# shahruk10/kaldi-tflite

Hardware: AMD Instinct MI355X
Metric: x-vectors/sec (10 s @16 kHz) (higher is better)
Workload: dtype f16mx

## Files before the change

kaldi-tflite_amd/csrc/tdnn_mx.hip:

```cpp
#include "tdnn_mx_common.h"

#define MXP_ROWS 256
__global__ __launch_bounds__(MXP_ROWS) void mx_planes_kernel(const float* __restrict__ src, int64_t T, int64_t ld, int D,
                                                             const int32_t* __restrict__ lens, char* __restrict__ xh,
                                                             char* __restrict__ xl4, char* __restrict__ x4, char* __restrict__ xs) {
    __shared__ float tile[MXP_ROWS * 33];
    const int b = blockIdx.z, c = blockIdx.y, nch = gridDim.y;
    const int64_t t0 = (int64_t)blockIdx.x * MXP_ROWS;
    const int64_t len = lens ? (int64_t)lens[b] : T;
    if (t0 >= len) return;
    const int rows = (int)(len - t0 < MXP_ROWS ? len - t0 : MXP_ROWS);
    const int tid = threadIdx.x;
    const float* base = src + ((int64_t)b * T + t0) * ld + c * 32;
    const bool vec = (ld & 3) == 0 && ((uintptr_t)src & 15) == 0 && c * 32 + 32 <= ld;
#pragma unroll
    for (int k = 0; k < 8; ++k) {
        const int q = k * MXP_ROWS + tid, r = q >> 3, e4 = (q & 7) * 4;
        if (r < rows) {
            float v[4];
            if (vec) {
                const f32x4 t = *reinterpret_cast<const f32x4*>(base + (int64_t)r * ld + e4);
                const int nd = D - (c * 32 + e4);
                v[0] = nd > 0 ? t.x : 0.0f; v[1] = nd > 1 ? t.y : 0.0f; v[2] = nd > 2 ? t.z : 0.0f; v[3] = nd > 3 ? t.w : 0.0f;
            } else {
#pragma unroll
                for (int e = 0; e < 4; ++e) v[e] = (c * 32 + e4 + e < D) ? base[(int64_t)r * ld + e4 + e] : 0.0f;
            }
#pragma unroll
            for (int e = 0; e < 4; ++e) tile[r * 33 + e4 + e] = __builtin_amdgcn_fmed3f(v[e], -65504.0f, 65504.0f);
        }
    }
    __syncthreads();
    const int64_t rec0 = ((int64_t)b * nch + c) * T + t0;
    u32x4 hp[4];
    if (tid < rows) {
        float v[32];
#pragma unroll
        for (int e = 0; e < 32; ++e) v[e] = tile[tid * 33 + e];
        u32x4 l4, h4;
        unsigned sw;
        mx_encode32(v, hp, l4, h4, sw);
        *reinterpret_cast<u32x4*>(xl4 + (rec0 + tid) * 16) = l4;
        *reinterpret_cast<u32x4*>(x4 + (rec0 + tid) * 16) = h4;
        *reinterpret_cast<unsigned*>(xs + (rec0 + tid) * 4) = sw;
    }
    __syncthreads();
    unsigned* himg = reinterpret_cast<unsigned*>(tile);
    if (tid < rows) {
#pragma unroll
        for (int k = 0; k < 4; ++k) *reinterpret_cast<u32x4*>(himg + tid * 20 + k * 4) = hp[k];
    }
    __syncthreads();
#pragma unroll
    for (int k = 0; k < 4; ++k) {
        const int q = k * MXP_ROWS + tid, r = q >> 2;
        if (r < rows)
            *reinterpret_cast<u32x4*>(xh + rec0 * 64 + (int64_t)q * 16) = *reinterpret_cast<const u32x4*>(himg + r * 20 + (q & 3) * 4);
    }
}

extern "C" int ktf_mx_planes(const float* src, int64_t B, int64_t T, int32_t D, int64_t ld_src, const int32_t* lens, void* xh,
                             void* xl4, void* x4, void* xs, void* stream) {
    KTF_REQUIRE(B >= 0 && T >= 0 && D > 0 && ld_src >= D, "ktf_mx_planes: bad size");
    if (B == 0 || T == 0) return KTF_OK;
    KTF_REQUIRE(src && xh && xl4 && x4 && xs, "ktf_mx_planes: null argument");
    const int nch = (D + 31) / 32;
    KTF_REQUIRE(B < 65536 && nch < 65536, "ktf_mx_planes: B and D / 32 must be below 65536");
    hipLaunchKernelGGL(mx_planes_kernel, dim3((unsigned)((T + MXP_ROWS - 1) / MXP_ROWS), (unsigned)nch, (unsigned)B), dim3(MXP_ROWS), 0,
                       (hipStream_t)stream, src, T, ld_src, (int)D, lens, (char*)xh, (char*)xl4, (char*)x4, (char*)xs);
    KTF_CHECK_LAUNCH("ktf_mx_planes");
    return KTF_OK;
}

template <int ACT, int OUT, bool PADK, bool FLAT = false>
__device__ __forceinline__ void mx_tile(const MxParams& p, const int id, int mtiles, int ntiles, int gtiles, double* __restrict__ stats,
                                        unsigned char* rsm) {
    static_assert(!FLAT || OUT != MX_OUT_F32, "flat row tiles: plane output or fused pooling");
#define MX_ARG_BATCH()                                                                                                                     \
    asm volatile("" ::"s"(p.xh), "s"(p.wh), "s"(p.T), "s"(p.nss), "s"(p.nk), "s"(p.nctx), "s"(p.nch_in), "s"(p.ctx_pk[0]), "s"(p.ctx_pk[1]), \
                 "s"(p.t_div_m), "s"(p.t_div_s), "s"(p.start), "s"(p.sub), "s"(p.cut))
    const int xcd = id & 7, slot = id >> 3;
    const int g = (slot / ntiles) * 8 + xcd;
    const int nt = slot - (slot / ntiles) * ntiles;
    if (g >= gtiles) return;
    const int b = FLAT ? 0 : g / mtiles, mt = FLAT ? g : g - b * mtiles;
    const int n0 = nt * 256, t0 = FLAT ? 0 : mt * 256;
    const int tid = threadIdx.x, lane = tid & 63;
    const int wave = __builtin_amdgcn_readfirstlane(tid >> 6);
    const int wm = wave >> 2, wn = wave & 3;
    const int R0 = mt * 256;
    int len, out_len;
    [[maybe_unused]] bool dense = false;
    if constexpr (FLAT) {
        const int total = p.row_starts[mtiles];
        MX_ARG_BATCH();
        if (R0 >= total) return;
        len = (int)p.T;
        out_len = total - R0 < 256 ? total - R0 : 256;
        dense = total == mtiles * len;
    } else {
        len = p.lens ? p.lens[b] : (int)p.T;
        MX_ARG_BATCH();
        out_len = len - p.cut - p.start <= 0 ? 0 : (len - p.cut - p.start + p.sub - 1) / p.sub;
        if (t0 >= out_len) return;
    }
    const int lenm1 = len - 1;
    const int64_t ub = FLAT ? 0 : (int64_t)b * p.nch_in * p.T;
    const int nkp = p.nss * 4;
    const __amdgpu_buffer_rsrc_t r_xh = mx_rsrc_pinned(p.xh + (ub - MX_KQ_BIAS) * 64);
    const __amdgpu_buffer_rsrc_t r_wh = mx_rsrc_pinned(p.wh + (int64_t)nt * nkp * MX_TILE);
    const __amdgpu_buffer_rsrc_t r_wq = mx_rsrc_pinned(p.wq + (int64_t)nt * p.nss * MX_WQ_BLOCK);

    unsigned a_cb[2];
    int a_row[2];
#pragma unroll
    for (int i = 0; i < 2; ++i) {
        const int q = i * 512 + tid;
        const int row = q >> 2;
        a_cb[i] = (unsigned)(((q & 3) ^ ((4 - ((row >> 2) & 3)) & 3)) * 16);
        a_row[i] = p.start + (t0 + row) * p.sub;
    }
    [[maybe_unused]] int a_lm1[2] = {lenm1, lenm1}, s_lm1 = lenm1;
    int s_row = p.start + (t0 + lane + 64 * (wave & 3)) * p.sub;
    [[maybe_unused]] unsigned a_ub[2] = {0u, 0u}, s_ub = 0u;
    [[maybe_unused]] auto flat_row = [&](int m) -> i32x4 {
        if (dense) {
            const int R = R0 + m;
            if (m >= out_len) return i32x4{-1, 0, 1, 0};
            const int bb = p.t_div_m ? (int)(__umulhi((unsigned)R, p.t_div_m) >> p.t_div_s) : R;
            return i32x4{R, R - bb * len, len, bb};
        }
        return reinterpret_cast<const i32x4*>(p.row_map)[R0 + m];
    };
    const unsigned long long cpk0 = p.ctx_pk[0], cpk1 = p.ctx_pk[1];
#define MX_CTX(ci_) ((int)(signed char)(((ci_) < 8 ? cpk0 : cpk1) >> (((ci_) & 7) * 8)))
    [[maybe_unused]] bool interior = false;
    if constexpr (FLAT) {
        i32x4 er[3];
        const int mr[3] = {tid >> 2, (512 + tid) >> 2, lane + 64 * (wave & 3)};
        if (dense) {
#pragma unroll
            for (int i = 0; i < 3; ++i) er[i] = flat_row(mr[i]);
        } else {
#pragma unroll
            for (int i = 0; i < 3; ++i) er[i] = reinterpret_cast<const i32x4*>(p.row_map)[R0 + mr[i]];
        }
#pragma unroll
        for (int i = 0; i < 2; ++i) {
            a_row[i] = er[i].y;
            a_lm1[i] = er[i].z - 1;
            a_ub[i] = er[i].x < 0 ? 0u : (unsigned)(er[i].x - er[i].y) * (unsigned)p.nch_in;
        }
        s_row = er[2].y;
        s_lm1 = er[2].z - 1;
        s_ub = er[2].x < 0 ? 0u : (unsigned)(er[2].x - er[2].y) * (unsigned)p.nch_in;
    }
    const unsigned vw = (unsigned)tid * 16u;
    const int wave_k0 = (int)(unsigned)(size_t)(lds_ptr_t*)(rsm + wave * 1024);
    [[maybe_unused]] const int wave_k = wave_k0;
#define MX_LDS_AT(off_, c_) ((lds_ptr_t*)(size_t)(unsigned)((off_) + (c_)))
    int kb[5], ko[5];
    kb[0] = MX_KQ_BIAS;
    ko[0] = MX_CTX(0);
#define MX_DMA_A_E(ks_, e_, n_)                                                                                        \
    {                                                                                                                  \
        int r_ = a_row[n_] + ko[e_];                                                                                   \
        const int hi_ = FLAT ? a_lm1[n_] : lenm1;                                                                      \
        r_ = r_ < 0 ? 0 : (r_ > hi_ ? hi_ : r_);                                                                       \
        const unsigned vo_ = ((FLAT ? a_ub[n_] : 0u) + (unsigned)r_) * 64u + a_cb[n_];                                 \
        __builtin_amdgcn_raw_ptr_buffer_load_lds(r_xh, MX_LDS_AT(wave_k, ((ks_) & 1) * MX_STAGE + (n_) * 8192), 16, vo_, kb[e_] << 6, 0, 0); \
    }
#define MX_DMA_A_I(ks_, e_, n_)                                                                                        \
    __builtin_amdgcn_raw_ptr_buffer_load_lds(r_xh, MX_LDS_AT(wave_k, ((ks_) & 1) * MX_STAGE + (n_) * 8192), 16, (n_) ? va1 : va0, \
                                             (kb[e_] + ko[e_]) << 6, 0, 0);
#define MX_DMA_A(ks_, e_, n_) { if constexpr (INTERIOR) MX_DMA_A_I(ks_, e_, n_) else MX_DMA_A_E(ks_, e_, n_) }
#define MX_DMA_W(ks_, n_)                                                                                              \
    __builtin_amdgcn_raw_ptr_buffer_load_lds(r_wh, MX_LDS_AT(wave_k, ((ks_) & 1) * MX_STAGE + MX_TILE + (n_) * 8192), 16, vw, \
                                             (ks_) * MX_TILE + (n_) * 8192, 0, 0);
    MX_DMA_W(0, 0) MX_DMA_W(0, 1) MX_DMA_A_E(0, 0, 0) MX_DMA_A_E(0, 0, 1)
    const __amdgpu_buffer_rsrc_t r_xl4 = mx_rsrc_pinned(p.xl4 + (ub - MX_KQ_BIAS) * 16);
    const __amdgpu_buffer_rsrc_t r_x4 = mx_rsrc_pinned(p.x4 + (ub - MX_KQ_BIAS) * 16);
    const __amdgpu_buffer_rsrc_t r_xs = mx_rsrc_pinned(p.xs + (ub - MX_KQ_BIAS) * 4);
    if constexpr (FLAT) {
        if (p.nctx == 1 && MX_CTX(0) == 0) {
            interior = true;
        } else if (out_len == 256) {
            const i32x4 e0 = flat_row(0), e1 = flat_row(255);
            interior = __builtin_amdgcn_readfirstlane(e0.w) == __builtin_amdgcn_readfirstlane(e1.w) &&
                       __builtin_amdgcn_readfirstlane(e0.y) + MX_CTX(0) >= 0 &&
                       __builtin_amdgcn_readfirstlane(e1.y) + MX_CTX(p.nctx - 1) <= __builtin_amdgcn_readfirstlane(e1.z) - 1;
        }
    }
    [[maybe_unused]] const unsigned va0 = (a_ub[0] + (unsigned)a_row[0]) * 64u + a_cb[0], va1 = (a_ub[1] + (unsigned)a_row[1]) * 64u + a_cb[1];
    [[maybe_unused]] const unsigned vs16 = (s_ub + (unsigned)s_row) * 16u, vs4 = (s_ub + (unsigned)s_row) * 4u;

    const int sa_k0 = (int)(unsigned)(size_t)(lds_ptr_t*)(rsm + (wave & 3) * 1024 + (wave >> 2) * 4096);
    const int sa_ks0 = (int)(unsigned)(size_t)(lds_ptr_t*)(rsm + (wave & 3) * 256 + (wave >> 2) * 1024);
    const bool wave_hi = wave >= 4;

    int* const tkb = reinterpret_cast<int*>(rsm + MX_KQ_OFF);
    int* const tko = tkb + (nkp + 4);

#define MX_DMA_SA(n_)                                                                                                  \
    {                                                                                                                  \
        constexpr int plane_ = ((n_) < 4 ? (n_) : 0) >> 1, h_ = (n_) < 4 ? ((n_) & 1) : (n_) - 4;                      \
        unsigned rec_ = 0u;                                                                                            \
        int so_;                                                                                                       \
        if constexpr (INTERIOR) {                                                                                      \
            so_ = sk_b[h_] + sk_o[h_];                                                                                 \
        } else {                                                                                                       \
            int r_ = s_row + sk_o[h_];                                                                                 \
            const int hi_ = FLAT ? s_lm1 : lenm1;                                                                      \
            r_ = r_ < 0 ? 0 : (r_ > hi_ ? hi_ : r_);                                                                   \
            rec_ = (FLAT ? s_ub : 0u) + (unsigned)r_;                                                                  \
            so_ = sk_b[h_];                                                                                            \
        }                                                                                                              \
        if ((n_) < 4) {                                                                                                \
            __builtin_amdgcn_raw_ptr_buffer_load_lds(plane_ ? r_x4 : r_xl4, MX_LDS_AT(sa_k, MX_SA_OFF + plane_ * 16384 + h_ * 8192), 16, \
                                                     INTERIOR ? vs16 : rec_ * 16u, so_ << 4, 0, 0);                    \
        } else {                                                                                                       \
            __builtin_amdgcn_raw_ptr_buffer_load_lds(r_xs, MX_LDS_AT(sa_ks, MX_SA_OFF + 32768 + h_ * 2048), 4, INTERIOR ? vs4 : rec_ * 4u, so_ << 2, 0, 0); \
        }                                                                                                              \
    }
#define MX_DMA_SW(ss_, n_)                                                                                             \
    __builtin_amdgcn_raw_ptr_buffer_load_lds(r_wq, MX_LDS_AT(wave_k, MX_SW_OFF + (n_) * 8192), 16, vw, (ss_) * MX_WQ_BLOCK + (n_) * 8192, 0, 0);

    f32x4 acc[8][4];
    const int r16 = lane & 15, q4 = lane >> 4;
    const int fr = (4 - ((r16 >> 2) & 3)) & 3;
    const int coff = ((q4 ^ fr) << 4);
    const int a_row_off = (wm * 128 + r16) * 64 + coff;
    const int b_row_off = (wn * 64 + r16) * 64 + coff;
    const int klim = PADK ? p.nk : nkp;

    auto kloop = [&](auto itag) {
        constexpr bool INTERIOR = decltype(itag)::value;
        {
            unsigned char* const prm_w = rsm + MX_PRM_OFF + (wave & 3) * 256;
            const unsigned vcol = (unsigned)(n0 + (wave & 3) * 64 + lane) * 4u;
            const float* const vec0 = wave_hi ? p.scale : p.bias;
            if (vec0) __builtin_amdgcn_raw_ptr_buffer_load_lds(mx_rsrc(vec0, p.units * 4), (lds_ptr_t*)(prm_w + (wave_hi ? 1024 : 0)), 4, vcol, 0, 0, 0);
            else reinterpret_cast<float*>(prm_w + (wave_hi ? 1024 : 0))[lane] = wave_hi ? 1.0f : 0.0f;
            if (!wave_hi) {
                if (p.shift) __builtin_amdgcn_raw_ptr_buffer_load_lds(mx_rsrc(p.shift, p.units * 4), (lds_ptr_t*)(prm_w + 2048), 4, vcol, 0, 0, 0);
                else reinterpret_cast<float*>(prm_w + 2048)[lane] = 0.0f;
            }
        }
        for (int k = tid; k < nkp + 4; k += 512) {
            const int kk = k + 1 < p.nk ? k + 1 : 0;
            const int ch = kk / p.nctx, ci = kk - ch * p.nctx;
            tkb[k] = ch * (int)p.T + MX_KQ_BIAS;
            tko[k] = MX_CTX(ci);
        }
        {
            int ch = 0, ci = 0;
#pragma unroll
            for (int e = 1; e <= 4; ++e) {
                if (++ci == p.nctx) { ci = 0; ++ch; }
                const bool real = e < p.nk;
                kb[e] = (real ? ch * (int)p.T : 0) + MX_KQ_BIAS;
                ko[e] = real ? MX_CTX(ci) : MX_CTX(0);
            }
        }
#pragma unroll
        for (int i = 0; i < 8; ++i)
#pragma unroll
            for (int j = 0; j < 4; ++j) acc[i][j] = f32x4{0.0f, 0.0f, 0.0f, 0.0f};
        for (int ss = 0; ss < p.nss; ++ss) {
            i32x4 tb_n, to_n;
            int sk_b[2], sk_o[2];
            int wave_k = wave_k0, sa_k = sa_k0, sa_ks = sa_ks0;
            asm volatile("" : "+s"(wave_k), "+s"(sa_k), "+s"(sa_ks));
#pragma unroll
            for (int j = 0; j < 4; ++j) {
                const int ks = 4 * ss + j;
                if (j == 1 || j == 2) asm volatile("s_waitcnt vmcnt(6)" ::: "memory");
                else if (j == 0) asm volatile("s_waitcnt vmcnt(0) lgkmcnt(0)" ::: "memory");
                else asm volatile("s_waitcnt vmcnt(0)" ::: "memory");
                __builtin_amdgcn_s_barrier();
                asm volatile("" ::: "memory");
                const bool live = PADK ? ks < p.nk : true;
#define MX_NEXT() ({ int k1_ = ks + 1; asm volatile("" : "+s"(k1_)); k1_ < klim; })
                const unsigned char* sa = rsm + (ks & 1) * MX_STAGE;
                const unsigned char* sw = sa + MX_TILE;
                hfrag8 bh[4];
                hfrag8 a_cur, a_nx1;
                if (live) {
#pragma unroll
                    for (int jj = 0; jj < 4; ++jj) bh[jj] = *reinterpret_cast<const hfrag8*>(sw + b_row_off + jj * 1024);
                    a_cur = *reinterpret_cast<const hfrag8*>(sa + a_row_off);
                    a_nx1 = *reinterpret_cast<const hfrag8*>(sa + a_row_off + 1024);
                }
                __builtin_amdgcn_sched_barrier(0);
                if (MX_NEXT()) { MX_DMA_A(ks + 1, j + 1, 0) MX_DMA_A(ks + 1, j + 1, 1) }
                __builtin_amdgcn_sched_barrier(0);
#pragma unroll
                for (int i = 0; i < 8; ++i) {
                    if (live) {
                        acc[i][0] = __builtin_amdgcn_mfma_f32_16x16x32_f16(a_cur, bh[0], acc[i][0], 0, 0, 0);
                        __builtin_amdgcn_sched_barrier(0);
                        hfrag8 a_nx2 = a_nx1;
                        if (i < 6) a_nx2 = *reinterpret_cast<const hfrag8*>(sa + a_row_off + (i + 2) * 1024);
#pragma unroll
                        for (int jj = 1; jj < 4; ++jj) acc[i][jj] = __builtin_amdgcn_mfma_f32_16x16x32_f16(a_cur, bh[jj], acc[i][jj], 0, 0, 0);
                        a_cur = a_nx1;
                        a_nx1 = a_nx2;
                    }
                    __builtin_amdgcn_sched_barrier(0);
                    if (i == 0) { if (MX_NEXT()) MX_DMA_W(ks + 1, 0) }
                    if (i == 1) { if (MX_NEXT()) MX_DMA_W(ks + 1, 1) }
                    if (j == 0) {
                        if (i == 1) {
                            sk_b[0] = wave_hi ? kb[1] : kb[0]; sk_o[0] = wave_hi ? ko[1] : ko[0];
                            sk_b[1] = wave_hi ? kb[3] : kb[2]; sk_o[1] = wave_hi ? ko[3] : ko[2];
                        }
                        if (i == 2) MX_DMA_SA(0)
                        if (i == 3) MX_DMA_SA(1)
                        if (i == 4) MX_DMA_SA(2)
                        if (i == 5) MX_DMA_SA(3)
                        if (i == 6) MX_DMA_SA(4)
                        if (i == 7) MX_DMA_SA(5)
                    }
                    if (j == 1) {
                        if (i == 2) MX_DMA_SW(ss, 0)
                        if (i == 3) MX_DMA_SW(ss, 1)
                        if (i == 4) MX_DMA_SW(ss, 2)
                        if (i == 5) MX_DMA_SW(ss, 3)
                        if (i == 6) MX_DMA_SW(ss, 4)
                        if (i == 7) MX_DMA_SW(ss, 5)
                    }
                    if (j == 2 && i == 3) {
                        tb_n = *reinterpret_cast<const i32x4*>(tkb + 4 * ss + 4);
                        to_n = *reinterpret_cast<const i32x4*>(tko + 4 * ss + 4);
                    }
                    __builtin_amdgcn_sched_barrier(0);
                }
#undef MX_NEXT
            }
            __builtin_amdgcn_sched_barrier(0);
            {
                int tl;
                asm volatile("v_mbcnt_lo_u32_b32 %0, -1, 0\n\tv_mbcnt_hi_u32_b32 %0, -1, %0" : "=v"(tl));
                const int sw_rec = ((tl & 63) >> 4) * 256 + wn * 64 + (tl & 15);
                const int sa_rec = ((tl & 63) >> 4) * 256 + wm * 128 + (tl & 15);
                unsigned o_a16 = MX_SA_OFF + sa_rec * 16, o_a4 = MX_SA_OFF + 32768 + sa_rec * 4;
                asm volatile("" : "+v"(o_a16), "+v"(o_a4));
                const unsigned char* const pa16 = rsm + o_a16;
                const unsigned char* const pa4 = rsm + o_a4;
                unsigned o_w16 = MX_SW_OFF + sw_rec * 16, o_w8 = MX_SW_OFF + 32768 + sw_rec * 8, o_w4 = MX_SW_OFF + 40960 + sw_rec * 4;
                asm volatile("" : "+v"(o_w16), "+v"(o_w8), "+v"(o_w4));
                const unsigned char* const pw16 = rsm + o_w16;
                const unsigned char* const pw8 = rsm + o_w8;
                const unsigned char* const pw4 = rsm + o_w4;
                u32x4 w4[4], wl6a[4];
                u32x2 wl6b[4];
                unsigned wsc[4];
#pragma unroll
                for (int jj = 0; jj < 4; ++jj) {
                    w4[jj] = *reinterpret_cast<const u32x4*>(pw16 + jj * 256);
                    wl6a[jj] = *reinterpret_cast<const u32x4*>(pw16 + 16384 + jj * 256);
                    wl6b[jj] = *reinterpret_cast<const u32x2*>(pw8 + jj * 128);
                    wsc[jj] = *reinterpret_cast<const unsigned*>(pw4 + jj * 64);
                }
                u32x4 l_n = *reinterpret_cast<const u32x4*>(pa16);
                u32x4 h_n = *reinterpret_cast<const u32x4*>(pa16 + 16384);
                unsigned s_n = *reinterpret_cast<const unsigned*>(pa4);
#pragma unroll
                for (int i = 0; i < 8; ++i) {
                    const u32x4 l = l_n, h = h_n;
                    const unsigned asc = s_n;
                    if (i < 7) {
                        l_n = *reinterpret_cast<const u32x4*>(pa16 + (i + 1) * 256);
                        h_n = *reinterpret_cast<const u32x4*>(pa16 + 16384 + (i + 1) * 256);
                        s_n = *reinterpret_cast<const unsigned*>(pa4 + (i + 1) * 64);
                    }
                    const i32x8 al = i32x8{(int)l.x, (int)l.y, (int)l.z, (int)l.w, 0, 0, 0, 0};
                    const i32x8 ah = i32x8{(int)h.x, (int)h.y, (int)h.z, (int)h.w, 0, 0, 0, 0};
#pragma unroll
                    for (int jj = 0; jj < 4; ++jj) {
                        const i32x8 bw = i32x8{(int)w4[jj].x, (int)w4[jj].y, (int)w4[jj].z, (int)w4[jj].w, 0, 0, 0, 0};
                        acc[i][jj] = __builtin_amdgcn_mfma_scale_f32_16x16x128_f8f6f4(al, bw, acc[i][jj], 4, 4, 0, asc, 0, wsc[jj]);
                    }
#pragma unroll
                    for (int jj = 0; jj < 4; ++jj) {
                        const i32x8 bw = i32x8{(int)wl6a[jj].x, (int)wl6a[jj].y, (int)wl6a[jj].z, (int)wl6a[jj].w, (int)wl6b[jj].x, (int)wl6b[jj].y, 0, 0};
                        acc[i][jj] = __builtin_amdgcn_mfma_scale_f32_16x16x128_f8f6f4(ah, bw, acc[i][jj], 4, 2, 1, asc, 1, wsc[jj]);
                    }
                    if (i == 3) {
                        kb[0] = kb[4];
                        ko[0] = ko[4];
#pragma unroll
                        for (int e = 0; e < 4; ++e) {
                            kb[e + 1] = __builtin_amdgcn_readfirstlane(tb_n[e]);
                            ko[e + 1] = __builtin_amdgcn_readfirstlane(to_n[e]);
                        }
                    }
                    __builtin_amdgcn_sched_barrier(0);
                }
            }
        }
    };
    if constexpr (FLAT) {
        if (interior) kloop(std::true_type{});
        else kloop(std::false_type{});
    } else {
        kloop(std::false_type{});
    }
#undef MX_DMA_A
#undef MX_DMA_A_E
#undef MX_DMA_A_I
#undef MX_DMA_W
#undef MX_DMA_SA
#undef MX_DMA_SW
#undef MX_ARG_BATCH
#undef MX_LDS_AT
#undef MX_CTX

#include "tdnn_mx_epilogue.inc"
}

template <int ACT, int OUT, bool PADK, bool FLAT = false>
__global__ __launch_bounds__(512) void tdnn_mx_kernel(MxParams p, int mtiles, int ntiles, int gtiles, double* __restrict__ stats) {
    extern __shared__ __attribute__((aligned(16))) unsigned char rsm[];
    mx_tile<ACT, OUT, PADK, FLAT>(p, blockIdx.x, mtiles, ntiles, gtiles, stats, rsm);
}

static int mx_launch(const void* xh, const void* xl4, const void* x4, const void* xs, int64_t B, int64_t T, const int32_t* lens,
                     const KtfTdnnDesc* d, const void* wh, const void* wq, const float* bias, const float* scale, const float* shift,
                     void* yh, void* yl4, void* y4, void* ys, float* yf, int64_t ldy, double* stats, void* stream, const char* who,
                     const int32_t* row_starts = nullptr, const int32_t* row_map = nullptr) {
    KTF_REQUIRE(d && wh && wq, "%s: null argument", who);
    KTF_REQUIRE(d->gemm == KTF_GEMM_F16MX, "%s: needs KTF_GEMM_F16MX", who);
    KTF_REQUIRE(B >= 0 && T >= 0 && B < 65536, "%s: bad size", who);
    KTF_REQUIRE(B == 0 || T == 0 || (xh && xl4 && x4 && xs), "%s: null argument", who);
    if (const int rc = tdnn_check_desc(d, scale, shift, who); rc != KTF_OK) return rc;
    KTF_REQUIRE(d->subsampling <= 64, "%s: subsampling %d outside [1,64]", who, d->subsampling);
    const bool plain = !d->valid && d->subsampling == 1;
    KTF_REQUIRE(plain || !stats, "%s: the fused pooling takes SAME padding without subsampling", who);
    KTF_REQUIRE(d->act == KTF_ACT_NONE || d->act == KTF_ACT_RELU, "%s: fuses ReLU or no activation", who);
    KTF_REQUIRE(T * (int64_t)d->din_pad * 2 < (1ll << 31) - (1ll << 20), "%s: T * din_pad too large", who);
    KTF_REQUIRE((((int64_t)d->din_pad / 32 * d->nctx + 3) / 4) * 4 <= MX_KQ_MAX_STEPS || (d->flags & KTF_TDNN_MX_LOADER), "%s: more than %d K-steps (din_pad / 32 * contexts)", who, MX_KQ_MAX_STEPS);
    if (B == 0 || T == 0 || ktf_tdnn_out_len(T, d) <= 0) return KTF_OK;
    const int outs = (yh ? 1 : 0) + (yf ? 1 : 0) + (stats ? 1 : 0);
    KTF_REQUIRE(outs == 1, "%s: exactly one of the plane / fp32 / pooled outputs", who);
    if (yh) KTF_REQUIRE(yl4 && y4 && ys, "%s: a plane output needs all four planes", who);
    if (yf) KTF_REQUIRE(ldy >= d->units, "%s: ldy < units", who);
    if (B == 0 || T == 0) return KTF_OK;
    MxParams p;
    memset(&p, 0, sizeof(p));
    p.xh = (const char*)xh; p.xl4 = (const char*)xl4; p.x4 = (const char*)x4; p.xs = (const char*)xs;
    p.lens = lens; p.wh = (const char*)wh; p.wq = (const char*)wq; p.bias = bias; p.scale = scale; p.shift = shift;
    p.yh = (char*)yh; p.yl4 = (char*)yl4; p.y4 = (char*)y4; p.ys = (char*)ys; p.yf = yf; p.ldy = ldy; p.T = T;
    p.units = d->units; p.nch_in = d->din_pad / 32; p.nctx = d->nctx; p.nk = p.nch_in * d->nctx; p.nss = (p.nk + 3) / 4;
    p.nch_out = (d->units + 31) / 32;
    p.sub = d->subsampling;
    p.start = (d->valid && d->ctx[0] < 0) ? -d->ctx[0] : 0;
    p.cut = (d->valid && d->ctx[d->nctx - 1] > 0) ? d->ctx[d->nctx - 1] : 0;
    p.Tout = ktf_tdnn_out_len(T, d);
    if (p.Tout <= 0) return KTF_OK;
    KTF_REQUIRE(plain || !(d->flags & KTF_TDNN_MX_LOADER), "%s: the loader-wave kernel takes SAME padding without subsampling", who);
    const bool loader = (d->flags & KTF_TDNN_MX_LOADER) != 0;
    const PoolSlots pool = (row_starts && !loader) ? pool_flat128() : pool_slots_mx(d->flags);
    p.stat_slots = (stats && (d->flags & KTF_TDNN_DET_STATS)) ? (int32_t)pool.slots(T) : 0;
    for (int i = 0; i < d->nctx; ++i) {
        KTF_REQUIRE(d->ctx[i] >= -128 && d->ctx[i] <= 127, "%s: context offsets outside [-128, 127]", who);
        p.ctx_pk[i >> 3] |= (unsigned long long)(unsigned char)(signed char)d->ctx[i] << ((i & 7) * 8);
    }
    hipStream_t st = (hipStream_t)stream;
    const int o = stats ? MX_OUT_STATS : (yf ? MX_OUT_F32 : MX_OUT_PLANES);
    if (loader) {
        const int rc = mxl_launch(p, B, d->act, o, stats, st);
        if (rc != KTF_OK) return rc;
        KTF_CHECK_LAUNCH(who);
        return KTF_OK;
    }
    if (row_starts) {
        KTF_REQUIRE(row_map && plain && o != MX_OUT_F32 && !loader, "%s: flat row tiles take the row table, SAME padding, no subsampling, a plane or pooled output", who);
        KTF_REQUIRE(B <= 4095 && B * T * (int64_t)p.nch_in * 64 < (1ll << 32) - (1ll << 20) && B * T < (1ll << 31) / (p.nch_out > 0 ? p.nch_out : 1),
                    "%s: flat row tiles need B <= 4095 and B * T * din_pad * 2 < 2^32", who);
        p.row_starts = row_starts; p.row_map = row_map;
        if (T > 1) {
            uint32_t l = 0;
            while ((1ull << l) < (uint64_t)T) ++l;
            p.t_div_m = (uint32_t)((1ull << (31 + l)) / (uint64_t)T + 1);
            p.t_div_s = l - 1;
        }
        const int ntiles = ktf_cdiv(d->units, 256);
        const int64_t ftiles = ktf_cdiv(B * T, 256);
        const int64_t fblocks = grouped_blocks(ftiles, ntiles);
        tdnn_pick<MX_OUT_STATS, MX_OUT_PLANES>(o, [&](auto O) {
            tdnn_pick<KTF_ACT_RELU, KTF_ACT_NONE>(d->act, [&](auto A) {
                tdnn_pick<true, false>((p.nk & 3) != 0, [&](auto PADK) {
                    tdnn_launch_kernel<tdnn_mx_kernel<A, O, PADK, true>>("tdnn_mx_kernel<flat>", dim3((unsigned)fblocks), dim3(512), MX_LDS_TOTAL(p.nss * 4),
                                                                         MX_LDS_TOTAL(MX_KQ_MAX_STEPS), st, p, (int)B, ntiles, (int)ftiles, stats);
                });
            });
        });
        KTF_CHECK_LAUNCH(who);
        return KTF_OK;
    }
    const int mtiles = ktf_cdiv(p.Tout, 256), ntiles = ktf_cdiv(d->units, 256);
    const int64_t gtiles = B * mtiles;
    const int64_t nblocks = grouped_blocks(gtiles, ntiles);
    tdnn_pick<KTF_ACT_RELU, KTF_ACT_NONE>(d->act, [&](auto A) {
        tdnn_pick<MX_OUT_STATS, MX_OUT_F32, MX_OUT_PLANES>(o, [&](auto O) {
            tdnn_pick<true, false>((p.nk & 3) != 0, [&](auto PADK) {
                tdnn_launch_kernel<tdnn_mx_kernel<A, O, PADK>>("tdnn_mx_kernel", dim3((unsigned)nblocks), dim3(512), MX_LDS_TOTAL(p.nss * 4),
                                                               MX_LDS_TOTAL(MX_KQ_MAX_STEPS), st, p, mtiles, ntiles, (int)gtiles, stats);
            });
        });
    });
    KTF_CHECK_LAUNCH(who);
    return KTF_OK;
}

extern "C" int ktf_tdnn_mx(const void* xh, const void* xl4, const void* x4, const void* xs, int64_t B, int64_t T, const int32_t* lens,
                           const KtfTdnnDesc* d, const void* wh, const void* wq, const float* bias, const float* scale,
                           const float* shift, void* yh, void* yl4, void* y4, void* ys, float* yf, int64_t ldy, void* stream) {
    return mx_launch(xh, xl4, x4, xs, B, T, lens, d, wh, wq, bias, scale, shift, yh, yl4, y4, ys, yf, ldy, nullptr, stream, "ktf_tdnn_mx");
}

extern "C" int ktf_tdnn_mx_flat(const void* xh, const void* xl4, const void* x4, const void* xs, int64_t B, int64_t T, const int32_t* row_starts,
                                const int32_t* row_map, const KtfTdnnDesc* d, const void* wh, const void* wq, const float* bias, const float* scale,
                                const float* shift, void* yh, void* yl4, void* y4, void* ys, void* stream) {
    KTF_REQUIRE(B == 0 || T == 0 || (row_starts && row_map && yh), "ktf_tdnn_mx_flat: null argument");
    return mx_launch(xh, xl4, x4, xs, B, T, nullptr, d, wh, wq, bias, scale, shift, yh, yl4, y4, ys, nullptr, 0, nullptr, stream, "ktf_tdnn_mx_flat",
                     row_starts, row_map);
}

extern "C" int ktf_tdnn_mx_flat_stats(const void* xh, const void* xl4, const void* x4, const void* xs, int64_t B, int64_t T, const int32_t* row_starts,
                                      const int32_t* row_map, const KtfTdnnDesc* d, const void* wh, const void* wq, const float* bias,
                                      const float* scale, const float* shift, double* sums, void* stream) {
    KTF_REQUIRE(sums && (B == 0 || T == 0 || (row_starts && row_map)), "ktf_tdnn_mx_flat_stats: null argument");
    return mx_launch(xh, xl4, x4, xs, B, T, nullptr, d, wh, wq, bias, scale, shift, nullptr, nullptr, nullptr, nullptr, nullptr, 0, sums, stream,
                     "ktf_tdnn_mx_flat_stats", row_starts, row_map);
}

extern "C" int ktf_tdnn_mx_stats(const void* xh, const void* xl4, const void* x4, const void* xs, int64_t B, int64_t T,
                                 const int32_t* lens, const KtfTdnnDesc* d, const void* wh, const void* wq, const float* bias,
                                 const float* scale, const float* shift, double* sums, void* stream) {
    KTF_REQUIRE(sums, "ktf_tdnn_mx_stats: null sums");
    return mx_launch(xh, xl4, x4, xs, B, T, lens, d, wh, wq, bias, scale, shift, nullptr, nullptr, nullptr, nullptr, nullptr, 0, sums, stream,
                     "ktf_tdnn_mx_stats");
}

extern "C" int32_t ktf_mx_slot_rows(int32_t flags) { return pool_slots_mx(flags).slot_rows; }
extern "C" int64_t ktf_mx_stats_slots(int64_t T, int32_t flags) { return pool_slots_mx(flags).slots(T); }
```

Before: 111,000.

## Add single-context flat MX TDNN kernel with arithmetic K offsets and early LDS reads

Adds a specialised flat-tile kernel for layers with a single zero-offset context (the 1x1 dense layers of the x-vector TDNN). It computes K-step offsets arithmetically instead of building and reading per-step offset tables in LDS, always takes the interior DMA path, and launches with the base LDS size only. It also moves the per-step LDS fragment reads for weights and activations into the tail of the previous DMA stage so they overlap with the issue of copies. The cost is another template instantiation and more live registers during the staging loop.

```diff
diff --git a/kaldi-tflite_amd/csrc/tdnn_mx.hip b/kaldi-tflite_amd/csrc/tdnn_mx.hip
--- a/kaldi-tflite_amd/csrc/tdnn_mx.hip
+++ b/kaldi-tflite_amd/csrc/tdnn_mx.hip
@@ -72,10 +72,11 @@
     return KTF_OK;
 }
 
-template <int ACT, int OUT, bool PADK, bool FLAT = false>
+template <int ACT, int OUT, bool PADK, bool FLAT = false, bool SINGLE = false>
 __device__ __forceinline__ void mx_tile(const MxParams& p, const int id, int mtiles, int ntiles, int gtiles, double* __restrict__ stats,
                                         unsigned char* rsm) {
     static_assert(!FLAT || OUT != MX_OUT_F32, "flat row tiles: plane output or fused pooling");
+    static_assert(!SINGLE || FLAT, "the single-context form is a flat-tile form");
 #define MX_ARG_BATCH()                                                                                                                     \
     asm volatile("" ::"s"(p.xh), "s"(p.wh), "s"(p.T), "s"(p.nss), "s"(p.nk), "s"(p.nctx), "s"(p.nch_in), "s"(p.ctx_pk[0]), "s"(p.ctx_pk[1]), \
                  "s"(p.t_div_m), "s"(p.t_div_s), "s"(p.start), "s"(p.sub), "s"(p.cut))
@@ -162,6 +163,9 @@
     int kb[5], ko[5];
     kb[0] = MX_KQ_BIAS;
     ko[0] = MX_CTX(0);
+    [[maybe_unused]] int kq_ss = MX_KQ_BIAS, tq_ss = (int)p.T;
+#define MX_KSO(e_) (SINGLE ? kq_ss + (e_) * tq_ss : kb[e_] + ko[e_])
+    [[maybe_unused]] const unsigned va0 = (a_ub[0] + (unsigned)a_row[0]) * 64u + a_cb[0], va1 = (a_ub[1] + (unsigned)a_row[1]) * 64u + a_cb[1];
 #define MX_DMA_A_E(ks_, e_, n_)                                                                                        \
     {                                                                                                                  \
         int r_ = a_row[n_] + ko[e_];                                                                                   \
@@ -172,16 +176,17 @@
     }
 #define MX_DMA_A_I(ks_, e_, n_)                                                                                        \
     __builtin_amdgcn_raw_ptr_buffer_load_lds(r_xh, MX_LDS_AT(wave_k, ((ks_) & 1) * MX_STAGE + (n_) * 8192), 16, (n_) ? va1 : va0, \
-                                             (kb[e_] + ko[e_]) << 6, 0, 0);
+                                             MX_KSO(e_) << 6, 0, 0);
 #define MX_DMA_A(ks_, e_, n_) { if constexpr (INTERIOR) MX_DMA_A_I(ks_, e_, n_) else MX_DMA_A_E(ks_, e_, n_) }
 #define MX_DMA_W(ks_, n_)                                                                                              \
     __builtin_amdgcn_raw_ptr_buffer_load_lds(r_wh, MX_LDS_AT(wave_k, ((ks_) & 1) * MX_STAGE + MX_TILE + (n_) * 8192), 16, vw, \
                                              (ks_) * MX_TILE + (n_) * 8192, 0, 0);
-    MX_DMA_W(0, 0) MX_DMA_W(0, 1) MX_DMA_A_E(0, 0, 0) MX_DMA_A_E(0, 0, 1)
+    MX_DMA_W(0, 0) MX_DMA_W(0, 1)
+    if constexpr (SINGLE) { MX_DMA_A_I(0, 0, 0) MX_DMA_A_I(0, 0, 1) } else { MX_DMA_A_E(0, 0, 0) MX_DMA_A_E(0, 0, 1) }
     const __amdgpu_buffer_rsrc_t r_xl4 = mx_rsrc_pinned(p.xl4 + (ub - MX_KQ_BIAS) * 16);
     const __amdgpu_buffer_rsrc_t r_x4 = mx_rsrc_pinned(p.x4 + (ub - MX_KQ_BIAS) * 16);
     const __amdgpu_buffer_rsrc_t r_xs = mx_rsrc_pinned(p.xs + (ub - MX_KQ_BIAS) * 4);
-    if constexpr (FLAT) {
+    if constexpr (FLAT && !SINGLE) {
         if (p.nctx == 1 && MX_CTX(0) == 0) {
             interior = true;
         } else if (out_len == 256) {
@@ -191,7 +196,6 @@
                        __builtin_amdgcn_readfirstlane(e1.y) + MX_CTX(p.nctx - 1) <= __builtin_amdgcn_readfirstlane(e1.z) - 1;
         }
     }
-    [[maybe_unused]] const unsigned va0 = (a_ub[0] + (unsigned)a_row[0]) * 64u + a_cb[0], va1 = (a_ub[1] + (unsigned)a_row[1]) * 64u + a_cb[1];
     [[maybe_unused]] const unsigned vs16 = (s_ub + (unsigned)s_row) * 16u, vs4 = (s_ub + (unsigned)s_row) * 4u;
 
     const int sa_k0 = (int)(unsigned)(size_t)(lds_ptr_t*)(rsm + (wave & 3) * 1024 + (wave >> 2) * 4096);
@@ -246,13 +250,15 @@
                 else reinterpret_cast<float*>(prm_w + 2048)[lane] = 0.0f;
             }
         }
-        for (int k = tid; k < nkp + 4; k += 512) {
-            const int kk = k + 1 < p.nk ? k + 1 : 0;
-            const int ch = kk / p.nctx, ci = kk - ch * p.nctx;
-            tkb[k] = ch * (int)p.T + MX_KQ_BIAS;
-            tko[k] = MX_CTX(ci);
-        }
-        {
+        if constexpr (!SINGLE) {
+            for (int k = tid; k < nkp + 4; k += 512) {
+                const int kk = k + 1 < p.nk ? k + 1 : 0;
+                const int ch = kk / p.nctx, ci = kk - ch * p.nctx;
+                tkb[k] = ch * (int)p.T + MX_KQ_BIAS;
+                tko[k] = MX_CTX(ci);
+            }
+        }
+        if constexpr (!SINGLE) {
             int ch = 0, ci = 0;
 #pragma unroll
             for (int e = 1; e <= 4; ++e) {
@@ -271,6 +277,43 @@
             int sk_b[2], sk_o[2];
             int wave_k = wave_k0, sa_k = sa_k0, sa_ks = sa_ks0;
             asm volatile("" : "+s"(wave_k), "+s"(sa_k), "+s"(sa_ks));
+            if constexpr (SINGLE) asm volatile("" : "+s"(tq_ss));
+            u32x4 w4[4], wl6a[4];
+            u32x2 wl6b[4];
+            unsigned wsc[4];
+            u32x4 l_n, h_n;
+            unsigned s_n;
+            const unsigned char *pa16, *pa4, *pw16, *pw8, *pw4;
+            auto m_addr = [&]() {
+                int tl;
+                asm volatile("v_mbcnt_lo_u32_b32 %0, -1, 0\n\tv_mbcnt_hi_u32_b32 %0, -1, %0" : "=v"(tl));
+                const int sw_rec = ((tl & 63) >> 4) * 256 + wn * 64 + (tl & 15);
+                const int sa_rec = ((tl & 63) >> 4) * 256 + wm * 128 + (tl & 15);
+                unsigned o_a16 = MX_SA_OFF + sa_rec * 16, o_a4 = MX_SA_OFF + 32768 + sa_rec * 4;
+                asm volatile("" : "+v"(o_a16), "+v"(o_a4));
+                pa16 = rsm + o_a16;
+                pa4 = rsm + o_a4;
+                unsigned o_w16 = MX_SW_OFF + sw_rec * 16, o_w8 = MX_SW_OFF + 32768 + sw_rec * 8, o_w4 = MX_SW_OFF + 40960 + sw_rec * 4;
+                asm volatile("" : "+v"(o_w16), "+v"(o_w8), "+v"(o_w4));
+                pw16 = rsm + o_w16;
+                pw8 = rsm + o_w8;
+                pw4 = rsm + o_w4;
+            };
+            auto m_read = [&](auto step) {
+                constexpr int S = decltype(step)::value;
+#pragma unroll
+                for (int jj = 0; jj < 4; ++jj) {
+                    if constexpr (S == 0) w4[jj] = *reinterpret_cast<const u32x4*>(pw16 + jj * 256);
+                    if constexpr (S == 1) wsc[jj] = *reinterpret_cast<const unsigned*>(pw4 + jj * 64);
+                    if constexpr (S == 2) wl6a[jj] = *reinterpret_cast<const u32x4*>(pw16 + 16384 + jj * 256);
+                    if constexpr (S == 3) wl6b[jj] = *reinterpret_cast<const u32x2*>(pw8 + jj * 128);
+                }
+                if constexpr (S == 1) {
+                    l_n = *reinterpret_cast<const u32x4*>(pa16);
+                    s_n = *reinterpret_cast<const unsigned*>(pa4);
+                }
+                if constexpr (S == 2) h_n = *reinterpret_cast<const u32x4*>(pa16 + 16384);
+            };
 #pragma unroll
             for (int j = 0; j < 4; ++j) {
                 const int ks = 4 * ss + j;
@@ -311,8 +354,17 @@
                     if (i == 1) { if (MX_NEXT()) MX_DMA_W(ks + 1, 1) }
                     if (j == 0) {
                         if (i == 1) {
-                            sk_b[0] = wave_hi ? kb[1] : kb[0]; sk_o[0] = wave_hi ? ko[1] : ko[0];
-                            sk_b[1] = wave_hi ? kb[3] : kb[2]; sk_o[1] = wave_hi ? ko[3] : ko[2];
+                            if constexpr (SINGLE) {
+                                const int blk = wave_hi ? 1 : 0;
+                                sk_b[0] = kq_ss + (wave_hi ? tq_ss : 0);
+                                sk_b[1] = sk_b[0] + 2 * tq_ss;
+                                if (PADK && 4 * ss + blk >= p.nk) sk_b[0] = MX_KQ_BIAS;
+                                if (PADK && 4 * ss + 2 + blk >= p.nk) sk_b[1] = MX_KQ_BIAS;
+                                sk_o[0] = sk_o[1] = 0;
+                            } else {
+                                sk_b[0] = wave_hi ? kb[1] : kb[0]; sk_o[0] = wave_hi ? ko[1] : ko[0];
+                                sk_b[1] = wave_hi ? kb[3] : kb[2]; sk_o[1] = wave_hi ? ko[3] : ko[2];
+                            }
                         }
                         if (i == 2) MX_DMA_SA(0)
                         if (i == 3) MX_DMA_SA(1)
@@ -329,7 +381,13 @@
                         if (i == 6) MX_DMA_SW(ss, 4)
                         if (i == 7) MX_DMA_SW(ss, 5)
                     }
-                    if (j == 2 && i == 3) {
+                    if (SINGLE && j == 3) {
+                        if (i == 4) { m_addr(); m_read(std::integral_constant<int, 0>{}); }
+                        if (i == 5) m_read(std::integral_constant<int, 1>{});
+                        if (i == 6) m_read(std::integral_constant<int, 2>{});
+                        if (i == 7) m_read(std::integral_constant<int, 3>{});
+                    }
+                    if (!SINGLE && j == 2 && i == 3) {
                         tb_n = *reinterpret_cast<const i32x4*>(tkb + 4 * ss + 4);
                         to_n = *reinterpret_cast<const i32x4*>(tko + 4 * ss + 4);
                     }
@@ -339,32 +397,19 @@
             }
             __builtin_amdgcn_sched_barrier(0);
             {
-                int tl;
-                asm volatile("v_mbcnt_lo_u32_b32 %0, -1, 0\n\tv_mbcnt_hi_u32_b32 %0, -1, %0" : "=v"(tl));
-                const int sw_rec = ((tl & 63) >> 4) * 256 + wn * 64 + (tl & 15);
-                const int sa_rec = ((tl & 63) >> 4) * 256 + wm * 128 + (tl & 15);
-                unsigned o_a16 = MX_SA_OFF + sa_rec * 16, o_a4 = MX_SA_OFF + 32768 + sa_rec * 4;
-                asm volatile("" : "+v"(o_a16), "+v"(o_a4));
-                const unsigned char* const pa16 = rsm + o_a16;
-                const unsigned char* const pa4 = rsm + o_a4;
-                unsigned o_w16 = MX_SW_OFF + sw_rec * 16, o_w8 = MX_SW_OFF + 32768 + sw_rec * 8, o_w4 = MX_SW_OFF + 40960 + sw_rec * 4;
-                asm volatile("" : "+v"(o_w16), "+v"(o_w8), "+v"(o_w4));
-                const unsigned char* const pw16 = rsm + o_w16;
-                const unsigned char* const pw8 = rsm + o_w8;
-                const unsigned char* const pw4 = rsm + o_w4;
-                u32x4 w4[4], wl6a[4];
-                u32x2 wl6b[4];
-                unsigned wsc[4];
-#pragma unroll
-                for (int jj = 0; jj < 4; ++jj) {
-                    w4[jj] = *reinterpret_cast<const u32x4*>(pw16 + jj * 256);
-                    wl6a[jj] = *reinterpret_cast<const u32x4*>(pw16 + 16384 + jj * 256);
-                    wl6b[jj] = *reinterpret_cast<const u32x2*>(pw8 + jj * 128);
-                    wsc[jj] = *reinterpret_cast<const unsigned*>(pw4 + jj * 64);
+                if constexpr (!SINGLE) {
+                    m_addr();
+#pragma unroll
+                    for (int jj = 0; jj < 4; ++jj) {
+                        w4[jj] = *reinterpret_cast<const u32x4*>(pw16 + jj * 256);
+                        wl6a[jj] = *reinterpret_cast<const u32x4*>(pw16 + 16384 + jj * 256);
+                        wl6b[jj] = *reinterpret_cast<const u32x2*>(pw8 + jj * 128);
+                        wsc[jj] = *reinterpret_cast<const unsigned*>(pw4 + jj * 64);
+                    }
+                    l_n = *reinterpret_cast<const u32x4*>(pa16);
+                    h_n = *reinterpret_cast<const u32x4*>(pa16 + 16384);
+                    s_n = *reinterpret_cast<const unsigned*>(pa4);
                 }
-                u32x4 l_n = *reinterpret_cast<const u32x4*>(pa16);
-                u32x4 h_n = *reinterpret_cast<const u32x4*>(pa16 + 16384);
-                unsigned s_n = *reinterpret_cast<const unsigned*>(pa4);
 #pragma unroll
                 for (int i = 0; i < 8; ++i) {
                     const u32x4 l = l_n, h = h_n;
@@ -386,7 +431,8 @@
                         const i32x8 bw = i32x8{(int)wl6a[jj].x, (int)wl6a[jj].y, (int)wl6a[jj].z, (int)wl6a[jj].w, (int)wl6b[jj].x, (int)wl6b[jj].y, 0, 0};
                         acc[i][jj] = __builtin_amdgcn_mfma_scale_f32_16x16x128_f8f6f4(ah, bw, acc[i][jj], 4, 2, 1, asc, 1, wsc[jj]);
                     }
-                    if (i == 3) {
+                    if (SINGLE && i == 3) kq_ss += 4 * tq_ss;
+                    if (!SINGLE && i == 3) {
                         kb[0] = kb[4];
                         ko[0] = ko[4];
 #pragma unroll
@@ -400,12 +446,15 @@
             }
         }
     };
-    if constexpr (FLAT) {
+    if constexpr (SINGLE) {
+        kloop(std::true_type{});
+    } else if constexpr (FLAT) {
         if (interior) kloop(std::true_type{});
         else kloop(std::false_type{});
     } else {
         kloop(std::false_type{});
     }
+#undef MX_KSO
 #undef MX_DMA_A
 #undef MX_DMA_A_E
 #undef MX_DMA_A_I
@@ -423,6 +472,11 @@
 __global__ __launch_bounds__(512) void tdnn_mx_kernel(MxParams p, int mtiles, int ntiles, int gtiles, double* __restrict__ stats) {
     extern __shared__ __attribute__((aligned(16))) unsigned char rsm[];
     mx_tile<ACT, OUT, PADK, FLAT>(p, blockIdx.x, mtiles, ntiles, gtiles, stats, rsm);
+}
+template <int ACT, int OUT, bool PADK>
+__global__ __launch_bounds__(512) void mx_single_kernel(MxParams p, int mtiles, int ntiles, int gtiles, double* __restrict__ stats) {
+    extern __shared__ __attribute__((aligned(16))) unsigned char rsm[];
+    mx_tile<ACT, OUT, PADK, true, true>(p, blockIdx.x, mtiles, ntiles, gtiles, stats, rsm);
 }
 
 static int mx_launch(const void* xh, const void* xl4, const void* x4, const void* xs, int64_t B, int64_t T, const int32_t* lens,
@@ -491,8 +545,12 @@
         tdnn_pick<MX_OUT_STATS, MX_OUT_PLANES>(o, [&](auto O) {
             tdnn_pick<KTF_ACT_RELU, KTF_ACT_NONE>(d->act, [&](auto A) {
                 tdnn_pick<true, false>((p.nk & 3) != 0, [&](auto PADK) {
-                    tdnn_launch_kernel<tdnn_mx_kernel<A, O, PADK, true>>("tdnn_mx_kernel<flat>", dim3((unsigned)fblocks), dim3(512), MX_LDS_TOTAL(p.nss * 4),
-                                                                         MX_LDS_TOTAL(MX_KQ_MAX_STEPS), st, p, (int)B, ntiles, (int)ftiles, stats);
+                    if (d->nctx == 1 && d->ctx[0] == 0)
+                        tdnn_launch_kernel<mx_single_kernel<A, O, PADK>>("tdnn_mx_kernel<flat>", dim3((unsigned)fblocks), dim3(512), MX_LDS_BYTES, MX_LDS_BYTES,
+                                                                         st, p, (int)B, ntiles, (int)ftiles, stats);
+                    else
+                        tdnn_launch_kernel<tdnn_mx_kernel<A, O, PADK, true>>("tdnn_mx_kernel<flat>", dim3((unsigned)fblocks), dim3(512), MX_LDS_TOTAL(p.nss * 4),
+                                                                             MX_LDS_TOTAL(MX_KQ_MAX_STEPS), st, p, (int)B, ntiles, (int)ftiles, stats);
                 });
             });
         });
```

After: 112,300, median of 6. 1.01x the previous value.
